# tgialoimtr/cnn_lstm_ctc_ocr

Measured on AMD Instinct MI355X. Metric: line-crops/sec (train step) at 32x256 bs=256; CER vs ref, higher is better.
Workload: dtype bf16

## Files before the change

cnn_lstm_ctc_ocr_amd/_lib.py:

```python
import ctypes
import os

import torch

_HERE = os.path.dirname(os.path.abspath(__file__))
LIB_PATH = os.environ.get("OCRK_LIB") or os.path.join(_HERE, "libocrk.so")

OCRK_OK = 0
OCRK_ERR_INVALID_ARG = 1
OCRK_ERR_HIP = 2
OCRK_ERR_INFEASIBLE = 3

F32 = 0
BF16 = 1

_p = ctypes.c_void_p
_i32 = ctypes.c_int
_u32 = ctypes.c_uint
_i64 = ctypes.c_int64
_f32 = ctypes.c_float
_sz = ctypes.c_size_t

SIGNATURES = {
    "ocrk_version": [],
# ... 86 lines not shown
    "ocrk_lstm_fwd_persistent_f32_workspace_size": [_i32, _i32],
    "ocrk_lstm_fwd_persistent_f32_flags_size": [_i32, _i32],
    "ocrk_lstm_fwd_persistent_f32": [_p, _p, _p, _i32, _i32, _i32, _p, _p, _p, _p, _p, _p, _p, _sz, _p],
    "ocrk_lstm_bwd_persistent_f32_supported": [_i32, _i32],
    "ocrk_lstm_bwd_persistent_f32_workspace_size": [_i32, _i32],
    "ocrk_lstm_bwd_persistent_f32": [_p, _p, _i32, _i32, _i32, _p, _p, _p, _p, _p, _p, _p, _p, _sz, _p],
    "ocrk_lstm_bwd_persistent_supported": [_i32, _i32],
    "ocrk_lstm_bwd_persistent_workspace_size": [_i32, _i32],
    "ocrk_lstm_bwd_persistent_slices": [_i32, _i32],
    "ocrk_lstm_bwd_persistent": [_p, _p, _i32, _i32, _i32, _p, _p, _p, _p, _p, _p, _p, _p, _sz, _p],
    "ocrk_lstm_fwd": [_p, _p, _p, _p, _p, _i32, _i32, _i32, _p, _p, _p, _p, _i32, _p],
    "ocrk_lstm_bwd": [_p, _p, _p, _p, _i32, _i32, _i32, _p, _p, _p, _p, _i32, _p],
    "ocrk_gemm_workspace_size": [_i32, _i32, _i32, _i32],
    "ocrk_gemm": [_i32, _i32, _i32, _i32, _i32, _f32, _p, _i64, _i64, _p, _i64, _i64, _p, _i64, _i64,
                  _i32, _p, _i32, _i32, _i32, _i32, _i32, _p, _sz, _p],
    "ocrk_adam": [_p, _p, _p, _p, _i64, _f32, _f32, _f32, _f32, _f32, _p],
    "ocrk_adam_ex": [_p, _p, _p, _p, _i64, _f32, _f32, _f32, _f32, _f32, _u32, _p],
    "ocrk_cast": [_p, _i32, _p, _i32, _i64, _p],
    "ocrk_split_bf16": [_p, _i64, _p, _p, _p],
    "ocrk_permute3": [_p, _i32, _i32, _i32, _i32, _p, _i32, _p],
    "ocrk_strided_copy": [_p, _i64, _i64, _i64, _i64, _p, _i32, _i64, _i64, _p],
    "ocrk_colsum_workspace_size": [_i64, _i32],
    "ocrk_colsum": [_p, _i64, _i32, _i32, _p, _i32, _p, _sz, _p],
    "ocrk_slab_sum_workspace_size": [_i32],
    "ocrk_slab_sum": [_p, _i32, _i32, _i32, _p, _i32, _p, _sz, _p],
    "ocrk_relu_mask": [_p, _p, _i64, _f32, _p, _i32, _p],
    "ocrk_mul_scalar": [_p, _i64, _p, _p],
    "ocrk_mean": [_p, _i32, _p, _p],
    "ocrk_seq_len": [_p, _i32, _p, _p],
    "ocrk_timer_create": [_p],
# ... 104 lines not shown
        call("ocrk_timer_record", self.h, stream_ptr())

    def elapsed_ms(self, end):
        ms = ctypes.c_float()
        call("ocrk_timer_elapsed", self.h, end.h, ctypes.byref(ms))
        return ms.value

    def __del__(self):
        if _lib is not None and self.h:
            _lib.ocrk_timer_destroy(self.h)


PROBES = {}


def call(name, *args):
    probe = PROBES.get(name)
    if probe is not None and probe[0] is not None and probe[0](args) is None:
        probe = None
    if probe is not None:
        work_fn, records = probe
        ev0, ev1 = Timer(), Timer()
        ev0.record()
        status = getattr(lib(), name)(*args)
        ev1.record()
        records.append((ev0, ev1, work_fn(args) if work_fn else 0.0))
    else:
        status = getattr(lib(), name)(*args)
    if status != OCRK_OK:
        msg = lib().ocrk_last_error().decode(errors="replace")
        if status in (OCRK_ERR_INFEASIBLE, OCRK_ERR_INVALID_ARG):
            raise InvalidArgumentError(status, msg)
        raise OcrkError(status, msg)
    return status


def ptr(t):
    return None if t is None else ctypes.c_void_p(t.data_ptr())


def stream_ptr(device=None):
# ... 2 lines not shown
```

cnn_lstm_ctc_ocr_amd/csrc/gemm.h:

```cpp
#pragma once
#include "common.h"

namespace ocrk {

enum AMode { A_ROWK = 0, A_COLK = 1, A_IM2COL = 2, A_IM2COL_FLIP = 3, A_IM2COL_T = 4 };
enum BMode { B_NK = 0, B_KN = 1 };

struct GemmParams {
    int M, N, K;
    int batch;
    const void* A; int64_t lda; int64_t strideA;
    const void* B; int64_t ldb; int64_t strideB;
    void* C; int64_t ldc; int64_t strideC;
    int c_bf16;
    const float* bias; int64_t strideBias;
    const void* mask; int64_t ldmask;
    int accumulate;
    int relu;
    float alpha;
    float* stats;
    float* splitk_ws;
    int splits;
    int k_chunk;
    int convH, convW, convC;
    int epi_staged;
    const void* mask_bits;
    void* relu_bits;
};

struct TileIdx { int bm, bn; bool valid; };
__device__ __forceinline__ TileIdx xcd_tile(int tm, int tn) {
    const int nT = tm * tn, per = (nT + 7) >> 3;
    const int t = (int)(blockIdx.x & 7) * per + (int)(blockIdx.x >> 3);
    if (t >= nT) return {0, 0, false};
    constexpr int GM = 4;
    const int gsz = GM * tn, grp = t / gsz, first = grp * GM;
    const int gm = min(GM, tm - first), w = t - grp * gsz;
    return {first + w % gm, w / gm, true};
}
__host__ __forceinline__ unsigned xcd_grid(int tm, int tn) { return 8u * (unsigned)((tm * tn + 7) / 8); }

int gemm(const GemmParams& p, int amode, int bmode, int dtype, hipStream_t stream);
// ... 16 lines not shown
```

cnn_lstm_ctc_ocr_amd/csrc/gemm.hip:

```cpp
#include <atomic>
#include <cstdlib>
#include <type_traits>

#include "gemm.h"
#include "mfma_util.h"

namespace ocrk {

template <int AM, typename CT>
__device__ __forceinline__ const CT* a_addr(const GemmParams& p, const CT* A, int m, int k, bool& ok) {
    if constexpr (AM == A_ROWK) {
        ok = m < p.M && k < p.K;
        return A + (int64_t)m * p.lda + k;
    } else if constexpr (AM == A_COLK) {
        ok = m < p.M && k < p.K;
        return A + (int64_t)k * p.lda + m;
    } else {
        int pix, kidx;
        if constexpr (AM == A_IM2COL_T) { pix = k; kidx = m; ok = k < p.K && m < p.M; }
        else { pix = m; kidx = k; ok = m < p.M && k < p.K; }
        const int C = p.convC, W = p.convW, H = p.convH;
        int tap = kidx / C, c = kidx - tap * C;
        int kh = tap / 3, kw = tap - kh * 3;
        int w = pix % W, t2 = pix / W, h = t2 % H, b = t2 / H;
// ... 565 lines not shown
    p.C = C; p.ldc = ldc; p.strideC = stride_c;
    p.c_bf16 = c_dtype == OCRK_BF16;
    p.bias = bias; p.strideBias = 0;
    p.relu = relu; p.accumulate = accumulate; p.alpha = alpha;
    p.splits = splits < 1 ? 1 : splits;
    int kc = (int)ocrk::cdiv(K, p.splits);
    p.k_chunk = (int)ocrk::cdiv(kc < 32 ? 32 : kc, 32) * 32;
    p.splits = (int)ocrk::cdiv(K > 0 ? K : 1, p.k_chunk);
    p.splitk_ws = (float*)ws;
    OCRK_REQUIRE(p.splits == 1 || ws_bytes >= ocrk::gemm_splitk_ws_bytes(M, N, p.batch, p.splits),
                 "ocrk_gemm: split-K workspace too small");
    int amode = trans_a ? ocrk::A_COLK : ocrk::A_ROWK;
    int bmode = trans_b ? ocrk::B_NK : ocrk::B_KN;
    return ocrk::gemm(p, amode, bmode, dtype, ocrk::as_stream(stream));
}
```

cnn_lstm_ctc_ocr_amd/csrc/gemm_pptn.hip:

```cpp
#include "gemm.h"
#include "mfma_util.h"

namespace ocrk {

namespace {

constexpr unsigned TT_OOB = 0x80000000u;

__device__ __forceinline__ void tt_dma16(const i32x4_t& r, void* lds, unsigned voff) {
    lds_dma16_asm(r, lds, voff);
}

__device__ __forceinline__ void tt_barrier() {
    asm volatile("" ::: "memory");
    __builtin_amdgcn_s_barrier();
    asm volatile("" ::: "memory");
}

template <int AM>
__global__ void __launch_bounds__(512) gemm_pptn_kernel(const GemmParams p) {
    constexpr int BM = 256, BN = 256, BK = 64, ROWB = 128, BLK = BK * ROWB;
    constexpr int A_BYTES = 4 * BLK, BUF = 8 * BLK;
    constexpr int NUA = 2, NUB = 2;
    extern __shared__ __attribute__((aligned(16))) char smem[];

    const int tid = threadIdx.x, lane = tid & 63;
    const int wave = __builtin_amdgcn_readfirstlane(tid >> 6);
    const int wm = wave >> 2, wn = wave & 3;
    const int i16 = lane & 15, g = lane >> 4;

    const int tm = (p.M + BM - 1) / BM, tn = (p.N + BN - 1) / BN;
    const int nT = tm * tn;
    const int nitems = nT * p.batch * p.splits;
    const int per = (nitems + 7) >> 3;
    const int w = (int)(blockIdx.x & 7) * per + (int)(blockIdx.x >> 3);
    if (w >= nitems || (int)(blockIdx.x >> 3) >= per) return;
    const int z = w / nT, t = w - z * nT;
    constexpr int GM = 4;
    const int gsz = GM * tn, grp = t / gsz, first = grp * GM;
    const int gm = min(GM, tm - first), rr = t - grp * gsz;
    const int m0 = (first + rr % gm) * BM, n0 = (rr / gm) * BN;
    const int zb = z / p.splits, zs = z - zb * p.splits;
    const bf16* A = reinterpret_cast<const bf16*>(p.A) + zb * p.strideA;
    const bf16* B = reinterpret_cast<const bf16*>(p.B) + zb * p.strideB;
    const int kbeg = zs * p.k_chunk;
    const int kend = min(p.K, kbeg + p.k_chunk);
    const int nk = max(1, (kend - kbeg + BK - 1) / BK);
    const i32x4_t ra = uniform_rsrc_words(A, (int64_t)p.K * (AM == A_IM2COL_T ? p.convC : p.lda) * 2);
    const i32x4_t rb = uniform_rsrc_words(B, (int64_t)p.K * p.ldb * 2);

    const int krow_l = (wave & 7) * 8 + (lane >> 3);
    const int chunk = (lane & 7) ^ (krow_l & 7);
    const int acol[4] = {0, 128, 64, 192};
    auto bcol = [&](int q, int pair) { return (2 * pair + (chunk >> 2)) * 64 + q * 32 + (chunk & 3) * 8; };
    const int bcols[4] = {bcol(0, 0), bcol(0, 1), bcol(1, 0), bcol(1, 1)};
    const unsigned a_lane = (unsigned)(((int64_t)krow_l * p.lda + m0 + 8 * chunk) * 2);
    const unsigned b_lane = (unsigned)(((int64_t)krow_l * p.ldb + n0) * 2);
    int t_dh[4] = {0, 0, 0, 0}, t_dw[4] = {0, 0, 0, 0}, t_c0[4] = {0, 0, 0, 0};
    if constexpr (AM == A_IM2COL_T) {
#pragma unroll
        for (int s = 0; s < 4; ++s) {
            const int col = min(m0 + acol[s], p.M - 1);
            const int tap = col / p.convC;
            t_dh[s] = tap / 3 - 1;
            t_dw[s] = tap % 3 - 1;
            t_c0[s] = col - tap * p.convC;
        }
    }

    auto issue = [&](auto U_, int kt, char* buf) {
        constexpr int U = decltype(U_)::value;
        const int k = kbeg + kt * BK + krow_l;
        const bool kok = k < kend;
        const unsigned kst = (unsigned)((int64_t)(kt * BK + kbeg) * (U == 0 || U == 3 ? p.lda : p.ldb) * 2);
        if constexpr ((U == 0 || U == 3) && AM == A_IM2COL_T) {
            const int pix_w = k % p.convW, pix_h = (k / p.convW) % p.convH;
#pragma unroll
            for (int i = 0; i < NUA; ++i) {
                const int s = (U == 0 ? 0 : 2) + i;
                const int hh = pix_h + t_dh[s], ww = pix_w + t_dw[s];
                const bool ok = kok && m0 + acol[s] + 8 * chunk < p.M && hh >= 0 && hh < p.convH && ww >= 0 &&
                                ww < p.convW;
                const int64_t off = ((int64_t)(k + t_dh[s] * p.convW + t_dw[s]) * p.convC + t_c0[s] + 8 * chunk) * 2;
                tt_dma16(ra, buf + (acol[s] / 64) * BLK + (wave & 7) * 1024, ok ? (unsigned)off : TT_OOB);
            }
        } else if constexpr (U == 0 || U == 3) {
#pragma unroll
            for (int i = 0; i < NUA; ++i) {
                const int s = (U == 0 ? 0 : 2) + i;
                const bool ok = kok && m0 + acol[s] + 8 * chunk < p.M;
                tt_dma16(ra, buf + (acol[s] / 64) * BLK + (wave & 7) * 1024, ok ? a_lane + kst + acol[s] * 2 : TT_OOB);
            }
        } else {
#pragma unroll
            for (int i = 0; i < NUB; ++i) {
                const int s = (U == 1 ? 0 : 2) + i;
                const int blk = (U == 1 ? 0 : 2) + i;
                const bool ok = kok && n0 + bcols[s] < p.N;
                tt_dma16(rb, buf + A_BYTES + blk * BLK + (wave & 7) * 1024,
                         ok ? b_lane + kst + (unsigned)(bcols[s] * 2) : TT_OOB);
            }
        }
    };

    floatx4 acc[8][4];
// ... 138 lines not shown
#endif
    if (!gemm_pptn_enabled() || M < 256 || N < nmin || M % 8 != 0 || N % 8 != 0) return false;
    if (amode == A_COLK) return true;
    return amode == A_IM2COL_T && convC % 64 == 0;
}

int gemm_pptn(const GemmParams& p, int amode, int bmode, int dtype, hipStream_t stream) {
    if (dtype != OCRK_BF16 || bmode != B_KN || !gemm_pptn_covers(amode, p.M, p.N, p.convC)) return -1;
    if (p.c_bf16 || p.bias || p.relu || p.mask || p.stats) return -1;
    if (p.ldb % 8 != 0 || (amode == A_COLK && p.lda % 8 != 0)) return -1;
    if (p.splits == 1 && (p.ldc % 4 != 0 || (uintptr_t)p.C % 16 != 0 || p.strideC % 4 != 0)) return -1;
    if (p.splits > 1 && (uintptr_t)p.splitk_ws % 16 != 0) return -1;
    const int64_t a_bytes = (int64_t)p.K * (amode == A_COLK ? p.lda : p.convC) * 2;
    if (a_bytes >= (1ll << 31) || (int64_t)p.K * p.ldb * 2 >= (1ll << 31)) return -1;
    if (amode == A_IM2COL_T && p.batch != 1) return -1;
    constexpr int LDS = 2 * 8 * 64 * 128;
    const void* kern = amode == A_COLK ? reinterpret_cast<const void*>(&gemm_pptn_kernel<A_COLK>)
                                       : reinterpret_cast<const void*>(&gemm_pptn_kernel<A_IM2COL_T>);
    static DeviceOnce configured[2];
    set_dyn_lds(configured[amode == A_COLK ? 0 : 1], kern, LDS);
    const int64_t items = cdiv(p.M, 256) * cdiv(p.N, 256) * (int64_t)p.batch * p.splits;
    const dim3 grid((unsigned)(cdiv(items, 8) * 8));
    if (amode == A_COLK) gemm_pptn_kernel<A_COLK><<<grid, 512, LDS, stream>>>(p);
    else gemm_pptn_kernel<A_IM2COL_T><<<grid, 512, LDS, stream>>>(p);
    return launch_status("gemm_pptn");
}

}
```

cnn_lstm_ctc_ocr_amd/csrc/lstm.hip:

```cpp
#include "gemm.h"
#include "recur.h"

using namespace ocrk;

__device__ __forceinline__ void stamp(long long* dbg, int i) {
    if (dbg && threadIdx.x == 0) {
        long long t = __builtin_amdgcn_s_memrealtime();
        dbg[(((int64_t)blockIdx.z * gridDim.y + blockIdx.y) * gridDim.x + blockIdx.x) * 8 + i] = t;
    }
}

template <typename CT, int BR, int HU>
__device__ __forceinline__ void lstm_fwd_epilogue(const float* __restrict__ sG, const int (&plen)[(BR * HU / 4 + 255) / 256],
                                                  const float (&pg)[(BR * HU / 4 + 255) / 256][4][4],
                                                  const float (&pc)[(BR * HU / 4 + 255) / 256][4],
                                                  const float (&ph)[(BR * HU / 4 + 255) / 256][4], int s, int B, int H,
                                                  int b0, int u0, int dir, float* __restrict__ c_state,
                                                  CT* __restrict__ h_out, CT* __restrict__ out,
                                                  CT* __restrict__ hprev_t, float* __restrict__ cprev_t,
                                                  CT* __restrict__ acts_t) {
    constexpr int UQ = HU / 4, EPQ4 = (BR * UQ + 255) / 256;
    constexpr bool EFULL = (BR * UQ) % 256 == 0;
    const int G4 = 4 * H;
#pragma unroll
// ... 9 lines not shown
        if (s < len) {
            const float* gl = sG + r * (4 * HU + 1) + u;
            float ai[4], aj[4], af[4], ao[4], c[4], h[4];
#pragma unroll
            for (int e = 0; e < 4; ++e) {
                ai[e] = sig_fast(gl[0 * HU + e] + pg[q][0][e]);
                aj[e] = tanh_fast(gl[1 * HU + e] + pg[q][1][e]);
                af[e] = sig_fast(gl[2 * HU + e] + pg[q][2][e] + 1.0f);
                ao[e] = sig_fast(gl[3 * HU + e] + pg[q][3][e]);
                c[e] = af[e] * pc[q][e] + ai[e] * aj[e];
                h[e] = ao[e] * tanh_fast(c[e]);
            }
            st4(c_state + st, c);
            st4(h_out + st, h);
            st4(out + ((int64_t)t * B + b) * 2 * H + dir * H + uu, h);
            st4(hprev_t + tb * H + uu, ph[q]);
            st4(cprev_t + tb * H + uu, pc[q]);
            st4(a + 0 * H, ai); st4(a + 1 * H, aj); st4(a + 2 * H, af); st4(a + 3 * H, ao);
        } else {
            const float z[4] = {0.f, 0.f, 0.f, 0.f};
            st4(h_out + st, ph[q]);
            st4(hprev_t + tb * H + uu, z);
            st4(cprev_t + tb * H + uu, z);
            st4(a + 0 * H, z); st4(a + 1 * H, z); st4(a + 2 * H, z); st4(a + 3 * H, z);
        }
    }
}

template <typename CT, int BR, int HU, int KC>
__global__ void __launch_bounds__(256)
lstm_fwd_step_kernel(const CT* __restrict__ gx, const CT* __restrict__ whT, const CT* __restrict__ h_in,
                     CT* __restrict__ h_out, float* __restrict__ c_state, const int* __restrict__ seq_len,
                     int s, int T, int B, int H, CT* __restrict__ out, CT* __restrict__ hprev_t,
                     float* __restrict__ cprev_t, CT* __restrict__ acts_t, long long* __restrict__ dbg) {
    using Core = RecurCore<CT, BR, 4 * HU, KC>;
    stamp(dbg, 0);
    __shared__ __attribute__((aligned(16))) char lds[Core::LDS_BYTES];
// ... 515 lines not shown
```

cnn_lstm_ctc_ocr_amd/csrc/lstm_persistent.hip:

```cpp
#include "common.h"
#include "mfma_util.h"
#include "persist.h"
#include "recur.h"

using namespace ocrk;

namespace {

__device__ __forceinline__ void pstamp(long long* dbg, int s, int i) {
    if (dbg && threadIdx.x == 0 && (s == 64 || (s == 65 && i == 0)))
        dbg[(int64_t)blockIdx.x * 8 + (s == 65 ? 6 : i)] = __builtin_amdgcn_s_memrealtime();
}

template <int NG>
__device__ __forceinline__ void bias_partials(float* part, const float (&bsum)[NG][4], float* red, int64_t slice_off,
                                              int H, int u0) {
    if (!part) return;
    constexpr int LDR = NG * PHU + 4;
    const int tid = threadIdx.x, er = tid >> 3, eu = 4 * (tid & 7);
    __syncthreads();
#pragma unroll
    for (int k = 0; k < NG; ++k)
#pragma unroll
        for (int e = 0; e < 4; ++e) red[er * LDR + k * PHU + eu + e] = bsum[k][e];
// ... 319 lines not shown
                ((unsigned long long)((unsigned)bf16_bits(hn[2]) | ((unsigned)bf16_bits(hn[3]) << 16)) << 32);
            put8((gu64*)(hx + obase), v, local);
        }
        asm volatile("s_waitcnt vmcnt(0)" ::: "memory");
        __syncthreads();
        if (tid == 0) raise_flag(gflags + member, base + (unsigned)(s + 1), local);
        pstamp(dbg, s, 4);

        const int64_t tb = ((int64_t)t * B + b0 + er) * 2 + dir;
        {
            float ov[4];
#pragma unroll
            for (int e = 0; e < 4; ++e) ov[e] = valid ? hn[e] : 0.f;
            st4(out + ((int64_t)t * B + b0 + er) * 2 * H + dir * H + u0 + eu, ov);
        }
        st4(hprev_t + tb * H + u0 + eu, hp);
        st4(cprev_t + tb * H + u0 + eu, cp);
#pragma unroll
        for (int k = 0; k < 4; ++k) st4(acts_t + tb * G4 + k * H + u0 + eu, a4[k]);
        pstamp(dbg, s, 5);
    }
}

constexpr int R16_ROWS = 16, R16_UNITS = 64;

__global__ void __launch_bounds__(512, 1)
lstm_fwd_r16_kernel(const bf16* __restrict__ gx, const bf16* __restrict__ whT, bf16* __restrict__ hx,
                    const int* __restrict__ seq_len, int T, int B, bf16* __restrict__ out, bf16* __restrict__ hprev_t,
                    float* __restrict__ cprev_t, bf16* __restrict__ acts_t, unsigned* __restrict__ flags,
                    unsigned* __restrict__ err, unsigned spin_limit) {
    constexpr int KS = 16, H = 512, G4 = 4 * H;
// ... 131 lines not shown
            return (unsigned)bf16_bits(x0) | ((unsigned)bf16_bits(x1) << 16);
        };

        {
            gu32* ph = (gu32*)(hx + ((int64_t)((s & 1) * 2 + dir) * B + b0 + er) * H + u0 + eu);
            const unsigned v = pack2(hn[0], hn[1]);
            if (local) *ph = v;
            else __hip_atomic_store(ph, v, __ATOMIC_RELAXED, __HIP_MEMORY_SCOPE_AGENT);
        }
        asm volatile("s_waitcnt vmcnt(0)" ::: "memory");
        __syncthreads();
        if (tid == 0) raise_flag(gflags + member, base + (unsigned)(s + 1), local);

        __builtin_nontemporal_store(valid ? pack2(hn[0], hn[1]) : 0u,
                                    reinterpret_cast<unsigned*>(out + ((int64_t)t * B + b0 + er) * 2 * H + dir * H + u0 + eu));
        __builtin_nontemporal_store(pack2(hp[0], hp[1]), reinterpret_cast<unsigned*>(hprev_t + tb * H + u0 + eu));
        __builtin_nontemporal_store(f32x2_t{cp[0], cp[1]}, reinterpret_cast<f32x2_t*>(cprev_t + tb * H + u0 + eu));
#pragma unroll
        for (int k = 0; k < 4; ++k)
            __builtin_nontemporal_store(pack2(a4[k][0], a4[k][1]),
                                        reinterpret_cast<unsigned*>(acts_t + tb * G4 + k * H + u0 + eu));
    }
}

template <int KS, bool LATE = false>
__global__ void __launch_bounds__(256, 1)
lstm_bwd_persistent_kernel(const bf16* __restrict__ wh, bf16* __restrict__ dzx, const int* __restrict__ seq_len,
                           int T, int B, const bf16* __restrict__ dout, const float* __restrict__ cprev_t,
                           const bf16* __restrict__ acts_t, bf16* __restrict__ dG_t, unsigned* __restrict__ flags,
                           unsigned* __restrict__ err, unsigned spin_limit, long long* __restrict__ dbg,
                           float* __restrict__ bpart) {
// ... 843 lines not shown
```

cnn_lstm_ctc_ocr_amd/kernels.py:

```python
import ctypes

import torch

from . import _lib, options
from ._lib import ptr, call

F32, BF16 = _lib.F32, _lib.BF16
_DT = {torch.float32: F32, torch.bfloat16: BF16}


def dtype_code(dt):
    try:
        return _DT[dt]
    except KeyError:
        raise TypeError(f"unsupported dtype {dt}; libocrk computes in float32 or bfloat16")


def _stream(t):
    return _lib.stream_ptr(t.device)


def _chk(*ts):
    for t in ts:
        if t is None:
# ... 457 lines not shown
    key = ("f32", B, H)
    if key not in _PERSISTENT:
        _PERSISTENT[key] = bool(_lib.lib().ocrk_lstm_fwd_persistent_f32_supported(B, H))
    return _PERSISTENT[key]


def lstm_f32_bwd_persistent_ok(B, H):
    if not options.get("LSTM_PERSISTENT") or f32_mode_exact():
        return False
    key = ("f32bwd", B, H)
    if key not in _PERSISTENT:
        _PERSISTENT[key] = bool(_lib.lib().ocrk_lstm_bwd_persistent_f32_supported(B, H))
    return _PERSISTENT[key]


def lstm_fwd(gx, whT, seq_len, T, B, H, dtype, save=True):
    _chk(gx, whT, seq_len)
    if gx.dtype != dtype or whT.dtype != dtype:
        raise TypeError(f"lstm_fwd: gx and whT must be {dtype} (got {gx.dtype}, {whT.dtype})")
    dev = gx.device
    if dtype == torch.float32 and lstm_f32_persistent_ok(B, H):
        out = torch.empty(T, B, 2 * H, dtype=dtype, device=dev)
        hprev = cprev = acts = None
        if save:
            hprev = torch.empty(T, B, 2, H, dtype=dtype, device=dev)
            cprev = torch.empty(T, B, 2, H, dtype=torch.float32, device=dev)
            acts = torch.empty(T, B, 2, 4 * H, dtype=dtype, device=dev)
        nb = _lib.lib().ocrk_lstm_fwd_persistent_f32_workspace_size(B, H)
        ws = _ws(nb, dev)
        call("ocrk_lstm_fwd_persistent_f32", ptr(gx), ptr(whT), ptr(seq_len), T, B, H, ptr(out), ptr(hprev),
             ptr(cprev), ptr(acts), ptr(lstm_error_word(dev)),
             ptr(persistent_flags("lstm_fwd_f32", B, H, dev, "ocrk_lstm_fwd_persistent_f32_flags_size")),
             ptr(ws), nb, _stream(gx))
        return out, hprev, cprev, acts
    if lstm_persistent_ok(B, H, dtype):
        out = torch.empty(T, B, 2 * H, dtype=dtype, device=dev)
        hprev = torch.empty(T, B, 2, H, dtype=dtype, device=dev)
        cprev = torch.empty(T, B, 2, H, dtype=torch.float32, device=dev)
        acts = torch.empty(T, B, 2, 4 * H, dtype=dtype, device=dev)
        nb = _lib.lib().ocrk_lstm_fwd_persistent_workspace_size(B, H)
        ws = _ws(nb, dev)
        call("ocrk_lstm_fwd_persistent", ptr(gx), ptr(whT), ptr(seq_len), T, B, H, ptr(out), ptr(hprev),
             ptr(cprev), ptr(acts), ptr(lstm_error_word(dev)), ptr(persistent_flags("lstm_fwd", B, H, dev)), ptr(ws),
             nb, _stream(gx))
        return out, hprev, cprev, acts
    h_state = torch.zeros(2, 2, B, H, dtype=dtype, device=dev)
    c_state = torch.zeros(2, B, H, dtype=torch.float32, device=dev)
    out = torch.zeros(T, B, 2 * H, dtype=dtype, device=dev)
    hprev = torch.empty(T, B, 2, H, dtype=dtype, device=dev)
    cprev = torch.empty(T, B, 2, H, dtype=torch.float32, device=dev)
    acts = torch.empty(T, B, 2, 4 * H, dtype=dtype, device=dev)
    call("ocrk_lstm_fwd", ptr(gx), ptr(whT), ptr(h_state), ptr(c_state), ptr(seq_len), T, B, H, ptr(out),
         ptr(hprev), ptr(cprev), ptr(acts), dtype_code(dtype), _stream(gx))
    return out, hprev, cprev, acts


def lstm_fused_x_ok(B, H, n_in, dtype):
    if not lstm_persistent_ok(B, H, dtype) or not hasattr(_lib.lib(), "ocrk_lstm_fwd_persistent_x_supported"):
        return False
    return bool(_lib.lib().ocrk_lstm_fwd_persistent_x_supported(B, H, n_in))


def lstm_fwd_fused_x(x, wxT, bias, whT, seq_len, T, B, H):
    _chk(x, wxT, bias, whT, seq_len)
    dev = x.device
    n_in = x.shape[-1]
    out = torch.empty(T, B, 2 * H, dtype=x.dtype, device=dev)
    hprev = torch.empty(T, B, 2, H, dtype=x.dtype, device=dev)
    cprev = torch.empty(T, B, 2, H, dtype=torch.float32, device=dev)
    acts = torch.empty(T, B, 2, 4 * H, dtype=x.dtype, device=dev)
    nb = _lib.lib().ocrk_lstm_fwd_persistent_workspace_size(B, H)
    ws = _ws(nb, dev)
    call("ocrk_lstm_fwd_persistent_x", ptr(x), n_in, ptr(wxT), ptr(bias), ptr(whT), ptr(seq_len), T, B, H, ptr(out),
         ptr(hprev), ptr(cprev), ptr(acts), ptr(lstm_error_word(dev)), ptr(persistent_flags("lstm_fwd_x", B, H, dev)),
         ptr(ws), nb, _stream(x))
    return out, hprev, cprev, acts


def lstm_bwd(wh, seq_len, dout, cprev, acts, T, B, H, dbias=None, defer=None):
    _chk(wh, seq_len, dout, cprev, acts, dbias)
    dtype = dout.dtype
    dev = dout.device
    dG = torch.empty(T, B, 2, 4 * H, dtype=dtype, device=dev)
    if dtype == torch.float32 and lstm_f32_bwd_persistent_ok(B, H):
        nb = _lib.lib().ocrk_lstm_bwd_persistent_f32_workspace_size(B, H)
        ws = _ws(nb, dev)
        part = torch.empty(B // 32, 2 * 4 * H, dtype=torch.float32, device=dev) if dbias is not None else None
        call("ocrk_lstm_bwd_persistent_f32", ptr(wh), ptr(seq_len), T, B, H, ptr(dout), ptr(cprev), ptr(acts),
             ptr(dG), ptr(lstm_error_word(dev)), ptr(persistent_flags("lstm_bwd_f32", B, H, dev)), ptr(part),
             ptr(ws), nb, _stream(dout))
        if dbias is not None:
# ... 345 lines not shown
```

cnn_lstm_ctc_ocr_amd/model.py:

```python
import contextlib

import numpy as np
import torch
import torch.distributed as dist

from . import kernels as K
from . import options
from .config import BN_EPS, BN_MOMENTUM, INFER, LAYER_PARAMS, POOLS, TRAIN, ModelConfig, rnn_size
from .params import ParamStore

layer_params = LAYER_PARAMS

_DEFAULT = []


@contextlib.contextmanager
def use_store(store):
    _DEFAULT.append(store)
    try:
        yield store
    finally:
        _DEFAULT.pop()


# ... 256 lines not shown
def _conv_side(store, *tensors):
    if not options.get("CONV_SIDE"):
        return contextlib.nullcontext()
    return side_work(store, *tensors)


class _BiLSTM(torch.autograd.Function):

    @staticmethod
    def forward(ctx, x, seq_len, store, layer, *variables):
        dt = store.cfg.dtype
        T, B, n_in = x.shape
        H = store.cfg.rnn_sizes[layer - 1]
        wxT, _wx, whT, _wh, bias = store.lstm_images(layer, dt)
        gx = K.gemm(x.view(T * B, n_in), wxT, trans_b=True, bias=bias, out_dtype=dt)
        out, hprev, cprev, acts = K.lstm_fwd(gx, whT, seq_len, T, B, H, dt, save=any(ctx.needs_input_grad))
        ctx.store, ctx.layer, ctx.H = store, layer, H
        ctx.save_for_backward(x, seq_len, hprev, cprev, acts)
        return out

    @staticmethod
    def backward(ctx, dout):
        store, layer, H = ctx.store, ctx.layer, ctx.H
        x, seq_len, hprev, cprev, acts = ctx.saved_tensors
        dt = store.cfg.dtype
        T, B, n_in = x.shape
        G4 = 4 * H
        dout = dout.contiguous()
        if dout.dtype != dt:
            dout = K.cast(dout, dt)
        _wxT, wx, _whT, wh, _bias = store.lstm_images(layer, dt)
        dG = K.lstm_bwd(wh, seq_len, dout, cprev, acts, T, B, H, dbias=store.flat_bias_pair_grad(layer))
        R = T * B
        dx = None
        pre = f"rnn/bdrnn{layer}"
        with side_work(store, x, hprev, dG):
            gf, gb = store.grads[f"{pre}/fw/lstm_cell/kernel"], store.grads[f"{pre}/bw/lstm_cell/kernel"]
            sk = gf.numel()
            if dt == torch.float32 and not K.f32_mode_exact():
                (xh, xl), (hh, hl), (gh, gl) = K.split_bf16(x), K.split_bf16(hprev), K.split_bf16(dG)
                passes = [(xh, hh, gh), (xh, hh, gl), (xl, hl, gh)]
            else:
                passes = [(x, hprev, dG)]
            if gb.data_ptr() == gf.data_ptr() + 4 * sk:
                for _xa, ha, ga in passes:
                    K.gemm(ha.view(R, 2 * H), ga.view(R, 2 * G4), trans_a=True, out=gf[n_in:], accumulate=True,
                           M=H, N=G4, K=R, lda=2 * H, ldb=2 * G4, ldc=G4, batch=2, stride_a=H, stride_b=G4,
                           stride_c=sk, splits=_splits(H, G4, R, batch=2, items=_tn_items(layer)))
                for xa, _ha, ga in passes:
                    K.gemm(xa, ga.view(R, 2 * G4), trans_a=True, out=gf, accumulate=True, M=n_in, N=G4, K=R,
                           lda=n_in, ldb=2 * G4, ldc=G4, batch=2, stride_a=0, stride_b=G4, stride_c=sk,
                           splits=_splits(n_in, G4, R, batch=2, items=_tn_items(layer)))
            else:
                for xa, ha, ga in passes:
                    dg = ga.view(R, 2 * G4)
                    for d, gk in enumerate((gf, gb)):
                        dgd = dg[:, d * G4:]
                        K.gemm(xa, dgd, trans_a=True, out=gk, accumulate=True, M=n_in, N=G4, K=R, lda=n_in,
                               ldb=2 * G4, ldc=G4, splits=_splits(n_in, G4, R, items=_tn_items(layer)))
# ... 63 lines not shown
            K.gemm(hp, dgg, trans_a=True, out=gk[n_in:], accumulate=True, M=H, N=G2, K=R, lda=2 * H,
                   ldb=2 * G3, ldc=G2, splits=_splits(H, G2, R, items=_tn_items(layer)))
            K.gemm(x, dgc, trans_a=True, out=ck, accumulate=True, M=n_in, N=H, K=R, lda=n_in,
                   ldb=2 * G3, ldc=H, splits=_splits(n_in, H, R, items=_tn_items(layer)))
            K.gemm(rhd, dgc, trans_a=True, out=ck[n_in:], accumulate=True, M=H, N=H, K=R, lda=2 * H,
                   ldb=2 * G3, ldc=H, splits=_splits(H, H, R, items=_tn_items(layer)))
        side.__exit__(None, None, None)
        dx = None
        if ctx.needs_input_grad[0]:
            dx = K.gemm(dG.view(R, 2 * G3), wx, trans_b=True, out_dtype=dt).view(T, B, n_in)
        return (dx,) + (None,) * (len(ctx.needs_input_grad) - 1)




def _tn_items(layer):
    if layer == 1:
        return options.get("TN_ITEMS_L1")
    return options.get("TN_ITEMS")


def _splits(M, N, Kdim, batch=1, items=None):
    if M >= 256 and N >= 256:
        tiles = -(-M // 256) * -(-N // 256) * batch
        return int(max(1, min((items or options.get("TN_ITEMS")) // tiles, Kdim // 1024)))
    tiles = -(-M // 128) * -(-N // 128) * batch
    return int(max(1, min(-(-512 // tiles), Kdim // 2048)))


class _Logits(torch.autograd.Function):

    @staticmethod
    def forward(ctx, x, store, *variables):
# ... 178 lines not shown
```

cnn_lstm_ctc_ocr_amd/options.py:

```python
import contextlib
import os

_HOST_DEFAULTS = {
    "LSTM_PERSISTENT": 1,
    "F32_TRAIN_EXACT": 0,
    "SIDE_STREAM": 1,
    "CONV_SIDE": 1,
    "CONV12_FUSED": 1,
    "RELU_BITS": 1,
    "POOLED_BN": 1,
    "CONV1_FUSED": 1,
    "CONV12_BWD": 1,
    "TN_ITEMS": 256,
    "TN_ITEMS_L1": 160,
}
KERNEL_OPTIONS = ("CONV_DIRECT", "CONV_ROWS", "CONV_ROWS_WIDE", "CONV_WGRAD_BLOCKS", "LSTM_SPIN_LIMIT",
                  "PERSIST_LATE", "LSTM_BWD_R16", "CTC_LDS",
                  "PP_PERSIST_NK", "NT_F32_EXACT", "NT_F32_MASK",
                  "NT_F32_X6", "BEAM_WAVE", "BN_BWD_BLOCKS", "BN_ROUTE", "BN_ROUTE_SEG", "BN_ROUTE_NCH", "CONV_TN_ITEMS", "CONV_TN4_ITEMS",
                  "CONV_WGRAD_CUS", "F32_MFMA", "GEMM_NT", "GEMM_NT_STAGED", "GEMM_PP", "GEMM_PPTN", "PP_MIN_N", "GEMM_TN",
                  "LSTM_DMA", "LSTM_BWD_DMA", "LSTM_FWD_R16", "NT_TAP_UNIFORM")


def _env_int(name, default):
    v = os.environ.get("OCRK_" + name)
    if v is None or v == "":
        return default
    try:
        return int(v)
# ... 46 lines not shown
```

include/ocrk.h:

```cpp
#ifndef OCRK_H_
#define OCRK_H_

#include <stddef.h>
#include <stdint.h>

#ifdef __cplusplus
extern "C" {
#endif

#define OCRK_ABI_VERSION 7

enum ocrk_status {
    OCRK_OK = 0,
    OCRK_ERR_INVALID_ARG = 1,
    OCRK_ERR_HIP = 2,
    OCRK_ERR_INFEASIBLE = 3
};

enum ocrk_dtype { OCRK_F32 = 0, OCRK_BF16 = 1 };

int ocrk_set_f32_gemm_mode(int mode);
int ocrk_f32_gemm_exact(void);

enum ocrk_device_status {
// ... 194 lines not shown
                            const void* dout, const void* hprev_t, const void* acts_t, void* dG_t, unsigned* err,
                            unsigned* flags, float* dbias_part, void* ws, size_t ws_bytes, void* stream);
size_t ocrk_persistent_flags_size(int B, int H);
int ocrk_lstm_fwd(const void* gx, const void* whT, void* h_state, float* c_state, const int* seq_len,
                  int T, int B, int H, void* out, void* hprev_t, float* cprev_t, void* acts_t, int dtype,
                  void* stream);
int ocrk_lstm_bwd(const void* wh, void* dg_state, float* dc_state, const int* seq_len, int T, int B, int H,
                  const void* dout, const float* cprev_t, const void* acts_t, void* dG_t, int dtype,
                  void* stream);

size_t ocrk_gemm_workspace_size(int M, int N, int batch, int splits);
int ocrk_gemm(int trans_a, int trans_b, int M, int N, int K, float alpha, const void* A, int64_t lda,
              int64_t stride_a, const void* B, int64_t ldb, int64_t stride_b, void* C, int64_t ldc,
              int64_t stride_c, int c_dtype, const float* bias, int relu, int accumulate, int batch,
              int dtype, int splits, void* ws, size_t ws_bytes, void* stream);

int ocrk_adam(float* p, const float* g, float* m, float* v, int64_t n, float lr_t, float beta1,
              float beta2, float eps, float grad_scale, void* stream);
#define OCRK_ADAM_ZERO_GRAD 1u
int ocrk_adam_ex(float* p, float* g, float* m, float* v, int64_t n, float lr_t, float beta1,
                 float beta2, float eps, float grad_scale, unsigned flags, void* stream);

int ocrk_copy_batch(const void* jobs, int njobs, int64_t total_tiles, void* stream);
int ocrk_cast(const void* in, int in_dtype, void* out, int out_dtype, int64_t n, void* stream);
int ocrk_permute3(const void* in, int in_dtype, int d0, int d1, int d2, void* out, int out_dtype,
                  void* stream);
int ocrk_strided_copy(const float* in, int64_t rows, int64_t cols, int64_t in_rs, int64_t in_cs, void* out,
                      int out_dtype, int64_t out_rs, int64_t out_cs, void* stream);
size_t ocrk_colsum_workspace_size(int64_t M, int N);
int ocrk_colsum(const void* in, int64_t M, int N, int dtype, float* out, int accumulate, void* ws,
// ... 22 lines not shown
```

Measured before the change: 53940.

## Derive LSTM hprev from shifted output rows in weight-gradient GEMM

Adds an LSTM weight-gradient entry point whose TN GEMM can read the recurrent input straight from the layer output, shifted by one timestep per direction, and can optionally take the x input as a leading M-slice. With the default mode the forward pass no longer writes a separate hprev tensor, which removes that store traffic and its memory. Backward now runs the h-part through the new path and the x-part as a separate GEMM. Fused and deferred modes exist but are off by default, and the boundary rows depend on zero-fill through an out-of-bounds mask.

```diff
diff --git a/cnn_lstm_ctc_ocr_amd/_lib.py b/cnn_lstm_ctc_ocr_amd/_lib.py
--- a/cnn_lstm_ctc_ocr_amd/_lib.py
+++ b/cnn_lstm_ctc_ocr_amd/_lib.py
@@ -124,6 +124,7 @@
     "ocrk_gemm_workspace_size": [_i32, _i32, _i32, _i32],
     "ocrk_gemm": [_i32, _i32, _i32, _i32, _i32, _f32, _p, _i64, _i64, _p, _i64, _i64, _p, _i64, _i64,
                   _i32, _p, _i32, _i32, _i32, _i32, _i32, _p, _sz, _p],
+    "ocrk_lstm_wgrad": [_p, _i32, _p, _i64, _i32, _p, _i32, _i32, _i32, _p, _i32, _i32, _p, _sz, _p],
     "ocrk_adam": [_p, _p, _p, _p, _i64, _f32, _f32, _f32, _f32, _f32, _p],
     "ocrk_adam_ex": [_p, _p, _p, _p, _i64, _f32, _f32, _f32, _f32, _f32, _u32, _p],
     "ocrk_cast": [_p, _i32, _p, _i32, _i64, _p],
@@ -258,9 +259,11 @@
 PROBES = {}
 
 
-def call(name, *args):
-    probe = PROBES.get(name)
-    if probe is not None and probe[0] is not None and probe[0](args) is None:
+def call(name, *args, probe_as=None):
+    probe, pargs = PROBES.get(name), args
+    if probe is None and probe_as is not None:
+        probe, pargs = PROBES.get(probe_as[0]), probe_as[1]
+    if probe is not None and probe[0] is not None and probe[0](pargs) is None:
         probe = None
     if probe is not None:
         work_fn, records = probe
@@ -268,7 +271,7 @@
         ev0.record()
         status = getattr(lib(), name)(*args)
         ev1.record()
-        records.append((ev0, ev1, work_fn(args) if work_fn else 0.0))
+        records.append((ev0, ev1, work_fn(pargs) if work_fn else 0.0))
     else:
         status = getattr(lib(), name)(*args)
     if status != OCRK_OK:
diff --git a/cnn_lstm_ctc_ocr_amd/csrc/gemm.h b/cnn_lstm_ctc_ocr_amd/csrc/gemm.h
--- a/cnn_lstm_ctc_ocr_amd/csrc/gemm.h
+++ b/cnn_lstm_ctc_ocr_amd/csrc/gemm.h
@@ -26,6 +26,9 @@
     int epi_staged;
     const void* mask_bits;
     void* relu_bits;
+    const void* A2; int64_t lda2; int64_t strideA2;
+    int m_split;
+    int64_t a2_shift0, a2_shift_step;
 };
 
 struct TileIdx { int bm, bn; bool valid; };
diff --git a/cnn_lstm_ctc_ocr_amd/csrc/gemm.hip b/cnn_lstm_ctc_ocr_amd/csrc/gemm.hip
--- a/cnn_lstm_ctc_ocr_amd/csrc/gemm.hip
+++ b/cnn_lstm_ctc_ocr_amd/csrc/gemm.hip
@@ -603,3 +603,34 @@
     int bmode = trans_b ? ocrk::B_NK : ocrk::B_KN;
     return ocrk::gemm(p, amode, bmode, dtype, ocrk::as_stream(stream));
 }
+
+extern "C" int ocrk_lstm_wgrad(const void* x, int n_in, const void* h, int64_t ld_h, int shift_rows,
+                               const void* dG, int T, int B, int H, float* dW, int accumulate, int splits,
+                               void* ws, size_t ws_bytes, void* stream) {
+    OCRK_REQUIRE(h && dG && dW, "ocrk_lstm_wgrad: null operand");
+    OCRK_REQUIRE(T > 0 && B > 0 && n_in > 0 && H > 0 && n_in % 256 == 0 && H % 256 == 0,
+                 "ocrk_lstm_wgrad: n_in=%d and H=%d must be multiples of 256 (T=%d B=%d)", n_in, H, T, B);
+    OCRK_REQUIRE(ld_h >= 2 * (int64_t)H && (shift_rows == 0 || shift_rows == B),
+                 "ocrk_lstm_wgrad: ld_h=%lld < 2H or shift_rows=%d not 0 or B", (long long)ld_h, shift_rows);
+    OCRK_REQUIRE((int64_t)T * B < (1ll << 31), "ocrk_lstm_wgrad: T*B exceeds 2^31 rows");
+    const int K = T * B, M = x ? n_in + H : H, N = 4 * H;
+    ocrk::GemmParams p = {};
+    p.M = M; p.N = N; p.K = K; p.batch = 2;
+    p.A = x ? x : h; p.lda = x ? n_in : ld_h; p.strideA = 0;
+    p.A2 = h; p.lda2 = ld_h; p.strideA2 = H; p.m_split = x ? n_in : 0;
+    p.a2_shift0 = -(int64_t)shift_rows; p.a2_shift_step = 2 * (int64_t)shift_rows;
+    p.B = dG; p.ldb = 2 * (int64_t)N; p.strideB = N;
+    p.C = x ? dW : dW + (int64_t)n_in * N; p.ldc = N; p.strideC = (int64_t)(n_in + H) * N;
+    p.accumulate = accumulate; p.alpha = 1.f;
+    p.splits = splits < 1 ? 1 : splits;
+    int kc = (int)ocrk::cdiv(K, p.splits);
+    p.k_chunk = (int)ocrk::cdiv(kc < 32 ? 32 : kc, 32) * 32;
+    p.splits = (int)ocrk::cdiv(K, p.k_chunk);
+    p.splitk_ws = (float*)ws;
+    OCRK_REQUIRE(p.splits == 1 || ws_bytes >= ocrk::gemm_splitk_ws_bytes(M, N, 2, p.splits),
+                 "ocrk_lstm_wgrad: split-K workspace too small");
+    hipStream_t st = ocrk::as_stream(stream);
+    const int rc = ocrk::gemm_pptn(p, ocrk::A_COLK, ocrk::B_KN, OCRK_BF16, st);
+    OCRK_REQUIRE(rc >= 0, "ocrk_lstm_wgrad: the TN engine does not cover n_in=%d H=%d T*B=%d", n_in, H, K);
+    return rc != OCRK_OK ? rc : ocrk::splitk_finish(p, st);
+}
diff --git a/cnn_lstm_ctc_ocr_amd/csrc/gemm_pptn.hip b/cnn_lstm_ctc_ocr_amd/csrc/gemm_pptn.hip
--- a/cnn_lstm_ctc_ocr_amd/csrc/gemm_pptn.hip
+++ b/cnn_lstm_ctc_ocr_amd/csrc/gemm_pptn.hip
@@ -17,8 +17,9 @@
     asm volatile("" ::: "memory");
 }
 
-template <int AM>
+template <int AM, bool TAIL = false>
 __global__ void __launch_bounds__(512) gemm_pptn_kernel(const GemmParams p) {
+    static_assert(!TAIL || AM == A_COLK, "the A tail is a k-major source");
     constexpr int BM = 256, BN = 256, BK = 64, ROWB = 128, BLK = BK * ROWB;
     constexpr int A_BYTES = 4 * BLK, BUF = 8 * BLK;
     constexpr int NUA = 2, NUB = 2;
@@ -41,12 +42,18 @@
     const int gm = min(GM, tm - first), rr = t - grp * gsz;
     const int m0 = (first + rr % gm) * BM, n0 = (rr / gm) * BN;
     const int zb = z / p.splits, zs = z - zb * p.splits;
-    const bf16* A = reinterpret_cast<const bf16*>(p.A) + zb * p.strideA;
+    const bool tail = TAIL && m0 >= p.m_split;
+    const bf16* A = tail ? reinterpret_cast<const bf16*>(p.A2) + zb * p.strideA2
+                         : reinterpret_cast<const bf16*>(p.A) + zb * p.strideA;
+    const int64_t lda_a = tail ? p.lda2 : p.lda;
+    const int m0a = tail ? m0 - p.m_split : m0;
+    const int ma = !TAIL ? p.M : tail ? p.M - p.m_split : p.m_split;
+    const int64_t a2_shift = tail ? p.a2_shift0 + zb * p.a2_shift_step : 0;
     const bf16* B = reinterpret_cast<const bf16*>(p.B) + zb * p.strideB;
     const int kbeg = zs * p.k_chunk;
     const int kend = min(p.K, kbeg + p.k_chunk);
     const int nk = max(1, (kend - kbeg + BK - 1) / BK);
-    const i32x4_t ra = uniform_rsrc_words(A, (int64_t)p.K * (AM == A_IM2COL_T ? p.convC : p.lda) * 2);
+    const i32x4_t ra = uniform_rsrc_words(A, (int64_t)p.K * (AM == A_IM2COL_T ? p.convC : lda_a) * 2);
     const i32x4_t rb = uniform_rsrc_words(B, (int64_t)p.K * p.ldb * 2);
 
     const int krow_l = (wave & 7) * 8 + (lane >> 3);
@@ -54,7 +61,7 @@
     const int acol[4] = {0, 128, 64, 192};
     auto bcol = [&](int q, int pair) { return (2 * pair + (chunk >> 2)) * 64 + q * 32 + (chunk & 3) * 8; };
     const int bcols[4] = {bcol(0, 0), bcol(0, 1), bcol(1, 0), bcol(1, 1)};
-    const unsigned a_lane = (unsigned)(((int64_t)krow_l * p.lda + m0 + 8 * chunk) * 2);
+    const unsigned a_lane = (unsigned)(((int64_t)krow_l * lda_a + m0a + 8 * chunk) * 2);
     const unsigned b_lane = (unsigned)(((int64_t)krow_l * p.ldb + n0) * 2);
     int t_dh[4] = {0, 0, 0, 0}, t_dw[4] = {0, 0, 0, 0}, t_c0[4] = {0, 0, 0, 0};
     if constexpr (AM == A_IM2COL_T) {
@@ -72,7 +79,7 @@
         constexpr int U = decltype(U_)::value;
         const int k = kbeg + kt * BK + krow_l;
         const bool kok = k < kend;
-        const unsigned kst = (unsigned)((int64_t)(kt * BK + kbeg) * (U == 0 || U == 3 ? p.lda : p.ldb) * 2);
+        const unsigned kst = (unsigned)((int64_t)(kt * BK + kbeg) * (U == 0 || U == 3 ? lda_a : p.ldb) * 2);
         if constexpr ((U == 0 || U == 3) && AM == A_IM2COL_T) {
             const int pix_w = k % p.convW, pix_h = (k / p.convW) % p.convH;
 #pragma unroll
@@ -84,11 +91,21 @@
                 const int64_t off = ((int64_t)(k + t_dh[s] * p.convW + t_dw[s]) * p.convC + t_c0[s] + 8 * chunk) * 2;
                 tt_dma16(ra, buf + (acol[s] / 64) * BLK + (wave & 7) * 1024, ok ? (unsigned)off : TT_OOB);
             }
-        } else if constexpr (U == 0 || U == 3) {
+        } else if constexpr ((U == 0 || U == 3) && TAIL) {
+            const int64_t ks = (int64_t)k + a2_shift;
+            const bool rok = kok && ks >= 0 && ks < p.K;
 #pragma unroll
             for (int i = 0; i < NUA; ++i) {
                 const int s = (U == 0 ? 0 : 2) + i;
-                const bool ok = kok && m0 + acol[s] + 8 * chunk < p.M;
+                const bool ok = rok && m0a + acol[s] + 8 * chunk < ma;
+                const int64_t off = (ks * lda_a + m0a + acol[s] + 8 * chunk) * 2;
+                tt_dma16(ra, buf + (acol[s] / 64) * BLK + (wave & 7) * 1024, ok ? (unsigned)off : TT_OOB);
+            }
+        } else if constexpr (U == 0 || U == 3) {
+#pragma unroll
+            for (int i = 0; i < NUA; ++i) {
+                const int s = (U == 0 ? 0 : 2) + i;
+                const bool ok = kok && m0a + acol[s] + 8 * chunk < ma;
                 tt_dma16(ra, buf + (acol[s] / 64) * BLK + (wave & 7) * 1024, ok ? a_lane + kst + acol[s] * 2 : TT_OOB);
             }
         } else {
@@ -257,14 +274,20 @@
     const int64_t a_bytes = (int64_t)p.K * (amode == A_COLK ? p.lda : p.convC) * 2;
     if (a_bytes >= (1ll << 31) || (int64_t)p.K * p.ldb * 2 >= (1ll << 31)) return -1;
     if (amode == A_IM2COL_T && p.batch != 1) return -1;
+    const bool tail = p.A2 != nullptr;
+    if (tail && (amode != A_COLK || p.m_split < 0 || p.m_split >= p.M || p.m_split % 256 != 0 ||
+                 (p.M - p.m_split) % 256 != 0 || p.lda2 % 8 != 0 || (int64_t)p.K * p.lda2 * 2 >= (1ll << 31)))
+        return -1;
     constexpr int LDS = 2 * 8 * 64 * 128;
-    const void* kern = amode == A_COLK ? reinterpret_cast<const void*>(&gemm_pptn_kernel<A_COLK>)
-                                       : reinterpret_cast<const void*>(&gemm_pptn_kernel<A_IM2COL_T>);
-    static DeviceOnce configured[2];
-    set_dyn_lds(configured[amode == A_COLK ? 0 : 1], kern, LDS);
+    const void* kern = tail             ? reinterpret_cast<const void*>(&gemm_pptn_kernel<A_COLK, true>)
+                       : amode == A_COLK ? reinterpret_cast<const void*>(&gemm_pptn_kernel<A_COLK>)
+                                         : reinterpret_cast<const void*>(&gemm_pptn_kernel<A_IM2COL_T>);
+    static DeviceOnce configured[3];
+    set_dyn_lds(configured[tail ? 2 : amode == A_COLK ? 0 : 1], kern, LDS);
     const int64_t items = cdiv(p.M, 256) * cdiv(p.N, 256) * (int64_t)p.batch * p.splits;
     const dim3 grid((unsigned)(cdiv(items, 8) * 8));
-    if (amode == A_COLK) gemm_pptn_kernel<A_COLK><<<grid, 512, LDS, stream>>>(p);
+    if (tail) gemm_pptn_kernel<A_COLK, true><<<grid, 512, LDS, stream>>>(p);
+    else if (amode == A_COLK) gemm_pptn_kernel<A_COLK><<<grid, 512, LDS, stream>>>(p);
     else gemm_pptn_kernel<A_IM2COL_T><<<grid, 512, LDS, stream>>>(p);
     return launch_status("gemm_pptn");
 }
diff --git a/cnn_lstm_ctc_ocr_amd/csrc/lstm.hip b/cnn_lstm_ctc_ocr_amd/csrc/lstm.hip
--- a/cnn_lstm_ctc_ocr_amd/csrc/lstm.hip
+++ b/cnn_lstm_ctc_ocr_amd/csrc/lstm.hip
@@ -47,13 +47,13 @@
             st4(c_state + st, c);
             st4(h_out + st, h);
             st4(out + ((int64_t)t * B + b) * 2 * H + dir * H + uu, h);
-            st4(hprev_t + tb * H + uu, ph[q]);
+            if (hprev_t) st4(hprev_t + tb * H + uu, ph[q]);
             st4(cprev_t + tb * H + uu, pc[q]);
             st4(a + 0 * H, ai); st4(a + 1 * H, aj); st4(a + 2 * H, af); st4(a + 3 * H, ao);
         } else {
             const float z[4] = {0.f, 0.f, 0.f, 0.f};
             st4(h_out + st, ph[q]);
-            st4(hprev_t + tb * H + uu, z);
+            if (hprev_t) st4(hprev_t + tb * H + uu, z);
             st4(cprev_t + tb * H + uu, z);
             st4(a + 0 * H, z); st4(a + 1 * H, z); st4(a + 2 * H, z); st4(a + 3 * H, z);
         }
diff --git a/cnn_lstm_ctc_ocr_amd/csrc/lstm_persistent.hip b/cnn_lstm_ctc_ocr_amd/csrc/lstm_persistent.hip
--- a/cnn_lstm_ctc_ocr_amd/csrc/lstm_persistent.hip
+++ b/cnn_lstm_ctc_ocr_amd/csrc/lstm_persistent.hip
@@ -357,7 +357,7 @@
             for (int e = 0; e < 4; ++e) ov[e] = valid ? hn[e] : 0.f;
             st4(out + ((int64_t)t * B + b0 + er) * 2 * H + dir * H + u0 + eu, ov);
         }
-        st4(hprev_t + tb * H + u0 + eu, hp);
+        if (hprev_t) st4(hprev_t + tb * H + u0 + eu, hp);
         st4(cprev_t + tb * H + u0 + eu, cp);
 #pragma unroll
         for (int k = 0; k < 4; ++k) st4(acts_t + tb * G4 + k * H + u0 + eu, a4[k]);
@@ -519,7 +519,8 @@
 
         __builtin_nontemporal_store(valid ? pack2(hn[0], hn[1]) : 0u,
                                     reinterpret_cast<unsigned*>(out + ((int64_t)t * B + b0 + er) * 2 * H + dir * H + u0 + eu));
-        __builtin_nontemporal_store(pack2(hp[0], hp[1]), reinterpret_cast<unsigned*>(hprev_t + tb * H + u0 + eu));
+        if (hprev_t)
+            __builtin_nontemporal_store(pack2(hp[0], hp[1]), reinterpret_cast<unsigned*>(hprev_t + tb * H + u0 + eu));
         __builtin_nontemporal_store(f32x2_t{cp[0], cp[1]}, reinterpret_cast<f32x2_t*>(cprev_t + tb * H + u0 + eu));
 #pragma unroll
         for (int k = 0; k < 4; ++k)
diff --git a/cnn_lstm_ctc_ocr_amd/kernels.py b/cnn_lstm_ctc_ocr_amd/kernels.py
--- a/cnn_lstm_ctc_ocr_amd/kernels.py
+++ b/cnn_lstm_ctc_ocr_amd/kernels.py
@@ -495,10 +495,12 @@
     return _PERSISTENT[key]
 
 
-def lstm_fwd(gx, whT, seq_len, T, B, H, dtype, save=True):
+def lstm_fwd(gx, whT, seq_len, T, B, H, dtype, save=True, save_hprev=True):
     _chk(gx, whT, seq_len)
     if gx.dtype != dtype or whT.dtype != dtype:
         raise TypeError(f"lstm_fwd: gx and whT must be {dtype} (got {gx.dtype}, {whT.dtype})")
+    if not save_hprev and dtype != torch.bfloat16:
+        raise ValueError("lstm_fwd: save_hprev=False is the bf16 path's (the fp32 BPTT route reads hprev)")
     dev = gx.device
     if dtype == torch.float32 and lstm_f32_persistent_ok(B, H):
         out = torch.empty(T, B, 2 * H, dtype=dtype, device=dev)
@@ -516,7 +518,7 @@
         return out, hprev, cprev, acts
     if lstm_persistent_ok(B, H, dtype):
         out = torch.empty(T, B, 2 * H, dtype=dtype, device=dev)
-        hprev = torch.empty(T, B, 2, H, dtype=dtype, device=dev)
+        hprev = torch.empty(T, B, 2, H, dtype=dtype, device=dev) if save_hprev else None
         cprev = torch.empty(T, B, 2, H, dtype=torch.float32, device=dev)
         acts = torch.empty(T, B, 2, 4 * H, dtype=dtype, device=dev)
         nb = _lib.lib().ocrk_lstm_fwd_persistent_workspace_size(B, H)
@@ -528,7 +530,7 @@
     h_state = torch.zeros(2, 2, B, H, dtype=dtype, device=dev)
     c_state = torch.zeros(2, B, H, dtype=torch.float32, device=dev)
     out = torch.zeros(T, B, 2 * H, dtype=dtype, device=dev)
-    hprev = torch.empty(T, B, 2, H, dtype=dtype, device=dev)
+    hprev = torch.empty(T, B, 2, H, dtype=dtype, device=dev) if save_hprev else None
     cprev = torch.empty(T, B, 2, H, dtype=torch.float32, device=dev)
     acts = torch.empty(T, B, 2, 4 * H, dtype=dtype, device=dev)
     call("ocrk_lstm_fwd", ptr(gx), ptr(whT), ptr(h_state), ptr(c_state), ptr(seq_len), T, B, H, ptr(out),
@@ -556,6 +558,31 @@
          ptr(hprev), ptr(cprev), ptr(acts), ptr(lstm_error_word(dev)), ptr(persistent_flags("lstm_fwd_x", B, H, dev)),
          ptr(ws), nb, _stream(x))
     return out, hprev, cprev, acts
+
+
+def lstm_wgrad_ok(n_in, H, dtype):
+    return dtype == torch.bfloat16 and n_in % 256 == 0 and H % 256 == 0
+
+
+def lstm_wgrad(x, h, dG, dW, T, B, H, shift_rows, splits=1, accumulate=True, n_in=None):
+    _chk(x, h, dG, dW)
+    n_in = x.shape[-1] if x is not None else n_in
+    R, N = T * B, 4 * H
+    M = n_in + H if x is not None else H
+    if (x is not None and x.numel() != R * n_in) or h.numel() != R * 2 * H or dG.numel() != R * 2 * N or \
+            dW.numel() != 2 * (n_in + H) * N:
+        raise ValueError("lstm_wgrad: operand sizes do not match T, B, H")
+    if any(t.dtype != torch.bfloat16 for t in (x, h, dG) if t is not None) or dW.dtype != torch.float32:
+        raise TypeError("lstm_wgrad: bf16 operands and an f32 gradient")
+    kc = -(-(-(-R // splits)) // 32) * 32 if splits > 1 else R
+    splits = -(-R // kc) if splits > 1 else 1
+    nb = _lib.lib().ocrk_gemm_workspace_size(M, N, 2, splits) if splits > 1 else 0
+    ws = _ws(nb, h.device) if nb else None
+    as_gemm = (1, 0, M, N, R, 1.0, ptr(x), n_in, 0, ptr(dG), 2 * N, N, ptr(dW), N, (n_in + H) * N, F32, None, 0,
+               int(accumulate), 2, BF16, splits, ptr(ws), nb, _stream(h))
+    call("ocrk_lstm_wgrad", ptr(x), n_in, ptr(h), 2 * H, int(shift_rows), ptr(dG), T, B, H, ptr(dW),
+         int(accumulate), splits, ptr(ws), nb, _stream(h), probe_as=("ocrk_gemm", as_gemm))
+    return dW
 
 
 def lstm_bwd(wh, seq_len, dout, cprev, acts, T, B, H, dbias=None, defer=None):
diff --git a/cnn_lstm_ctc_ocr_amd/model.py b/cnn_lstm_ctc_ocr_amd/model.py
--- a/cnn_lstm_ctc_ocr_amd/model.py
+++ b/cnn_lstm_ctc_ocr_amd/model.py
@@ -294,14 +294,19 @@
         H = store.cfg.rnn_sizes[layer - 1]
         wxT, _wx, whT, _wh, bias = store.lstm_images(layer, dt)
         gx = K.gemm(x.view(T * B, n_in), wxT, trans_b=True, bias=bias, out_dtype=dt)
-        out, hprev, cprev, acts = K.lstm_fwd(gx, whT, seq_len, T, B, H, dt, save=any(ctx.needs_input_grad))
-        ctx.store, ctx.layer, ctx.H = store, layer, H
-        ctx.save_for_backward(x, seq_len, hprev, cprev, acts)
+        pre = f"rnn/bdrnn{layer}"
+        gf, gb = store.grads[f"{pre}/fw/lstm_cell/kernel"], store.grads[f"{pre}/bw/lstm_cell/kernel"]
+        adjacent = gb.data_ptr() == gf.data_ptr() + 4 * gf.numel()
+        wgrad = options.get("LSTM_WGRAD") if adjacent and K.lstm_wgrad_ok(n_in, H, dt) else 0
+        out, hprev, cprev, acts = K.lstm_fwd(gx, whT, seq_len, T, B, H, dt, save=any(ctx.needs_input_grad),
+                                             save_hprev=wgrad not in (1, 2))
+        ctx.store, ctx.layer, ctx.H, ctx.wgrad = store, layer, H, wgrad
+        ctx.save_for_backward(x, seq_len, out if wgrad in (1, 2) else hprev, cprev, acts)
         return out
 
     @staticmethod
     def backward(ctx, dout):
-        store, layer, H = ctx.store, ctx.layer, ctx.H
+        store, layer, H, wgrad = ctx.store, ctx.layer, ctx.H, ctx.wgrad
         x, seq_len, hprev, cprev, acts = ctx.saved_tensors
         dt = store.cfg.dtype
         T, B, n_in = x.shape
@@ -314,15 +319,39 @@
         R = T * B
         dx = None
         pre = f"rnn/bdrnn{layer}"
-        with side_work(store, x, hprev, dG):
-            gf, gb = store.grads[f"{pre}/fw/lstm_cell/kernel"], store.grads[f"{pre}/bw/lstm_cell/kernel"]
-            sk = gf.numel()
+        gf, gb = store.grads[f"{pre}/fw/lstm_cell/kernel"], store.grads[f"{pre}/bw/lstm_cell/kernel"]
+        sk = gf.numel()
+        shift = B if wgrad in (1, 2) else 0
+        dW = gf.as_strided((2, n_in + H, G4), (sk, G4, 1)) if wgrad else None
+
+        def fused():
+            K.lstm_wgrad(x, hprev, dG, dW, T, B, H, shift,
+                         splits=_splits(n_in + H, G4, R, batch=2, items=_tn_items(layer, fused=True)))
+
+        if wgrad in (2, 3) and layer > 1 and options.get("LSTM_WGRAD_LATE"):
+            store.conv_late.append((fused, (x, hprev, dG)))
+            late = True
+        else:
+            late = False
+        with contextlib.nullcontext() if late else side_work(store, x, hprev, dG, *_conv_late_tensors(store)):
+            if not late:
+                _conv_late_run(store)
             if dt == torch.float32 and not K.f32_mode_exact():
                 (xh, xl), (hh, hl), (gh, gl) = K.split_bf16(x), K.split_bf16(hprev), K.split_bf16(dG)
                 passes = [(xh, hh, gh), (xh, hh, gl), (xl, hl, gh)]
             else:
                 passes = [(x, hprev, dG)]
-            if gb.data_ptr() == gf.data_ptr() + 4 * sk:
+            if late:
+                pass
+            elif wgrad in (2, 3):
+                fused()
+            elif wgrad == 1:
+                K.lstm_wgrad(None, hprev, dG, dW, T, B, H, shift, n_in=n_in,
+                             splits=_splits(H, G4, R, batch=2, items=_tn_items(layer)))
+                K.gemm(x, dG.view(R, 2 * G4), trans_a=True, out=gf, accumulate=True, M=n_in, N=G4, K=R,
+                       lda=n_in, ldb=2 * G4, ldc=G4, batch=2, stride_a=0, stride_b=G4, stride_c=sk,
+                       splits=_splits(n_in, G4, R, batch=2, items=_tn_items(layer)))
+            elif gb.data_ptr() == gf.data_ptr() + 4 * sk:
                 for _xa, ha, ga in passes:
                     K.gemm(ha.view(R, 2 * H), ga.view(R, 2 * G4), trans_a=True, out=gf[n_in:], accumulate=True,
                            M=H, N=G4, K=R, lda=2 * H, ldb=2 * G4, ldc=G4, batch=2, stride_a=H, stride_b=G4,
@@ -416,9 +445,9 @@
 
 
 
-def _tn_items(layer):
+def _tn_items(layer, fused=False):
     if layer == 1:
-        return options.get("TN_ITEMS_L1")
+        return options.get("TN_ITEMS_L1_FUSED" if fused else "TN_ITEMS_L1")
     return options.get("TN_ITEMS")
 
 
diff --git a/cnn_lstm_ctc_ocr_amd/options.py b/cnn_lstm_ctc_ocr_amd/options.py
--- a/cnn_lstm_ctc_ocr_amd/options.py
+++ b/cnn_lstm_ctc_ocr_amd/options.py
@@ -11,8 +11,11 @@
     "POOLED_BN": 1,
     "CONV1_FUSED": 1,
     "CONV12_BWD": 1,
+    "LSTM_WGRAD": 1,
+    "LSTM_WGRAD_LATE": 1,
     "TN_ITEMS": 256,
     "TN_ITEMS_L1": 160,
+    "TN_ITEMS_L1_FUSED": 192,
 }
 KERNEL_OPTIONS = ("CONV_DIRECT", "CONV_ROWS", "CONV_ROWS_WIDE", "CONV_WGRAD_BLOCKS", "LSTM_SPIN_LIMIT",
                   "PERSIST_LATE", "LSTM_BWD_R16", "CTC_LDS",
diff --git a/include/ocrk.h b/include/ocrk.h
--- a/include/ocrk.h
+++ b/include/ocrk.h
@@ -232,6 +232,9 @@
               int64_t stride_a, const void* B, int64_t ldb, int64_t stride_b, void* C, int64_t ldc,
               int64_t stride_c, int c_dtype, const float* bias, int relu, int accumulate, int batch,
               int dtype, int splits, void* ws, size_t ws_bytes, void* stream);
+int ocrk_lstm_wgrad(const void* x, int n_in, const void* h, int64_t ld_h, int shift_rows, const void* dG,
+                    int T, int B, int H, float* dW, int accumulate, int splits, void* ws, size_t ws_bytes,
+                    void* stream);
 
 int ocrk_adam(float* p, const float* g, float* m, float* v, int64_t n, float lr_t, float beta1,
               float beta2, float eps, float grad_scale, void* stream);
```

Result: no change. 54150, median of 6 (+0.4%).
